# geloescht/mxnet-maintenance

Hardware: AMD Instinct MI355X
Metric: images/sec (whole node) ResNet-50 fp16 batch 256/GPU at 1/2/4/8 MI355X (higher is better)
Workload: dtype fp16; 1 GPU; model=ResNet-50 v1b, global_batch=256, per_gpu_batch=256, image_size=224, parallelism=dp1, layout=NHWC, optimizer=mp-SGD momentum 0.9, lr 0.1 (linear warm-up 40 steps), hip_graph=True, deterministic=True

## Files before the change

mxnet_maintenance_amd/ops/kernel_fns.py:

```python
import os

import torch

from . import kernels as _K
from .. import _state
from ..utils import env as _env

__all__ = ['BatchNormNHWC', 'BatchNormDualTailNHWC', 'SoftmaxCE', 'GlobalAvgPoolNHWC', 'flat_sgd']

_DT = {torch.float32: 0, torch.float16: 1, torch.bfloat16: 2}


def _stream():
    return torch.cuda.current_stream().cuda_stream


def _p(t):
    return 0 if t is None else t.data_ptr()


def _f32(t):
    if t.dtype == torch.float32 and t.is_contiguous():
        return t
    m = getattr(t, '_mxamd_master', None)
# ... 93 lines not shown
        C = x.shape[-1]
        R = x.numel() // C
        dev = x.device
        assert pool is None or (relu and addend is None)
        y = torch.empty_like(x) if pool is None else None
        if addend is not None:
            assert addend.shape == x.shape and addend.dtype == x.dtype
            addend = addend.contiguous()
        g, mean, invstd, var, scale, shift, args, host_update = _bn_fwd_stats(
            lib, x, gamma, beta, moving_mean, moving_var, eps, training, momentum)
        mask = (torch.empty(x.numel() // 8, dtype=torch.uint8, device=dev)
                if (addend is not None and relu and _RELU_FROM_X[0]) else None)
        lib.bn_nhwc_forward(_DT[x.dtype], x.data_ptr(), _p(addend), _p(y), _p(mask), *args(relu))
        if host_update is not None:
            host_update()
        ctx.pool = None
        if pool is not None:
            (kh, kw), (sh, sw), (ph, pw) = pool
            N, H, W = x.shape[:3]
            Ho, Wo = _pool_out(H, kh, sh, ph, False), _pool_out(W, kw, sw, pw, False)
            y = torch.empty((N, Ho, Wo, C), dtype=x.dtype, device=dev)
            arg = torch.empty((N, Ho, Wo, C), dtype=torch.uint8, device=dev)
            ctx.pool = (N, H, W, C, Ho, Wo, kh, kw, sh, sw, ph, pw, 1)
            lib.pool_nhwc_forward_bnrelu(_DT[x.dtype], x.data_ptr(), y.data_ptr(), arg.data_ptr(), *ctx.pool,
                                         _stream(), scale.data_ptr(), shift.data_ptr())
            mask = arg
        relu_mode = 0 if not relu else (1 if not _RELU_FROM_X[0] else (3 if addend is not None else 2))
        if pool is not None:
            relu_mode = 2
        ctx.save_for_backward(x, y if relu_mode == 1 else mask, g, mean, invstd,
                              scale if relu_mode == 2 else None, shift if relu_mode == 2 else None)
        ctx.cfg = (relu_mode, bool(training), addend is not None, gamma.dtype, beta.dtype)
        ctx.tee_key = getattr(addend, '_mxamd_tee_key', None) if (addend is not None and relu_mode == 3) else None
        ctx.bn_token = None
        if training and relu_mode in (0, 2, 3) and _BN_BWD_FUSE[0] and pool is None:
            ctx.bn_token = _BnToken()
            y._mxamd_bn_src = (x, mean, scale if relu_mode == 2 else None, shift if relu_mode == 2 else None,
                               mask if relu_mode == 3 else None, relu_mode, ctx.bn_token)
        ctx.refs = (gamma, beta)
        ctx.add_src = None
        if relu_mode == 3 and training and _BN_BWD_FUSE[0] and _BN_TAIL_DS[0]:
            src = getattr(addend, '_mxamd_bn_src', None)
            if (src is not None and src[5] == 0 and tuple(src[0].shape) == tuple(x.shape)
                    and src[0].dtype == x.dtype and src[0].is_contiguous()):
                ctx.add_src = src
        third = invstd if (invstd_out and training) else var
        ctx.mark_non_differentiable(mean, third)
        ctx.set_materialize_grads(False)
        return y, mean, third

    @staticmethod
    def backward(ctx, gy, _gm, _gv):
        lib = _K.lib()
        x, y, g, mean, invstd, fscale, fshift = ctx.saved_tensors
        relu_mode, training, has_add, gdt, bdt = ctx.cfg
        gamma_ref, beta_ref = ctx.refs
        if gy is None:
            return (None,) * 12
        gy = gy.contiguous()
        C = x.shape[-1]
        R = x.numel() // C
        dev = x.device
        fused_pool = False
        if ctx.pool is not None:
            fused_pool = (x.dtype in (torch.float16, torch.bfloat16) and 256 % (C // 8) == 0
                          and hasattr(lib, 'bn_pool_backward') and _BN_POOL_BWD[0])
            if not fused_pool:
                gyd = torch.empty_like(x)
                lib.pool_nhwc_backward(_DT[x.dtype], 1, gy.data_ptr(), y.data_ptr(), gyd.data_ptr(), *ctx.pool,
                                       _stream())
                gy, y = gyd, None
        lazy_mask = None
        tok = ctx.bn_token
        if tok is not None and tok.lazy is not None:
            dy_l, mask_l, ver_l = tok.lazy
            tok.lazy = None
            if gy is dy_l and gy._version == ver_l and relu_mode == 0 and not has_add and ctx.pool is None:
                lazy_mask = mask_l
            else:
                gy = (gy - dy_l + _materialize_dz(dy_l, mask_l)).contiguous()
        dx = torch.empty_like(x)
        dz = torch.empty_like(x) if has_add else None
        ext = getattr(gy, '_mxamd_bn_bwd', None)
        ext_nblk = 0
        if (ext is not None and ctx.bn_token is not None and ext[2] is ctx.bn_token
                and ext[3] == gy._version):
            part, ext_nblk = ext[0], ext[1]
        else:
            nblk = lib.bn_partials_rows(R, C)
            part = torch.empty(2 * nblk * C, dtype=torch.float32, device=dev)
        out = torch.empty(5, C, dtype=torch.float32, device=dev)
        need_g, need_b = ctx.needs_input_grad[1], ctx.needs_input_grad[2]
        tg = _leaf_grad(gamma_ref, C) if need_g else None
        tb = _leaf_grad(beta_ref, C) if need_b else None
        direct = tb is not None and (tg is not None or not need_g) and (tg is not None or tb is not None)
        if direct:
            dg_buf = tg if tg is not None else torch.zeros(C, dtype=torch.float32, device=dev)
            dg_ptr, db_ptr, accum = dg_buf.data_ptr(), tb.data_ptr(), 1
        else:
            dg_ptr, db_ptr, accum = out[0].data_ptr(), out[1].data_ptr(), 0
        if fused_pool:
            N_, H_, W_, C_, Ho_, Wo_, kh, kw, sh, sw, ph, pw, _ = ctx.pool
            ppart = torch.empty(2 * lib.bn_pool_bwd_blocks() * C, dtype=torch.float32, device=dev)
            lib.bn_pool_backward(_DT[x.dtype], x.data_ptr(), gy.data_ptr(), y.data_ptr(), dx.data_ptr(), g.data_ptr(),
                                 mean.data_ptr(), invstd.data_ptr(), fscale.data_ptr(), fshift.data_ptr(),
                                 ppart.data_ptr(), dg_ptr, db_ptr, out[2].data_ptr(), N_, H_, W_, C_, Ho_, Wo_, kh, kw,
                                 sh, sw, ph, pw, 0, int(training), accum, _stream())
            if direct:
                return dx, None, None, None, None, None, None, None, None, None, None, None
            return (dx, out[0].to(gdt) if need_g else None, out[1].to(bdt) if need_b else None,
                    None, None, None, None, None, None, None, None, None)
        ymask = y if relu_mode == 3 else None
        y = y if relu_mode == 1 else None
        ds = ctx.add_src if dz is not None else None
        lazy = (dz is not None and ds is None and ymask is not None and ctx.tee_key is not None
                and lazy_shortcut_ok(ctx.tee_key))
        lazy_ds = (dz is not None and ds is not None and ymask is not None and _LAZY_DZ[0]
                   and isinstance(ds[6], _BnToken))
        if lazy or lazy_ds:
            dz = None
        kmode = relu_mode
        if lazy_mask is not None:
            kmode, ymask = 3, lazy_mask
        dkw = {}
        if ds is not None:
            ds_nblk = lib.bn_tail_ds_rows(R, C)
            ds_part = torch.empty(2 * ds_nblk * C, dtype=torch.float32, device=dev)
            dkw = dict(ds_z=ds[0].data_ptr(), ds_mean=ds[1].data_ptr(), ds_part=ds_part.data_ptr())
        lib.bn_nhwc_backward(_DT[x.dtype], x.data_ptr(), gy.data_ptr(), _p(y), _p(ymask), dx.data_ptr(), _p(dz),
                             g.data_ptr(),
                             mean.data_ptr(), invstd.data_ptr(), _p(fscale), _p(fshift), part.data_ptr(), dg_ptr,
                             db_ptr, out[2].data_ptr(), R, C, kmode, 0, int(training), accum, _stream(),
                             ext_nblk, **dkw)
        if ds is not None:
            if lazy_ds:
                gy._mxamd_bn_bwd = (ds_part, ds_nblk, ds[6], gy._version)
                ds[6].lazy = (gy, ymask, gy._version)
                dz = gy
            else:
                dz._mxamd_bn_bwd = (ds_part, ds_nblk, ds[6], dz._version)
        if lazy:
            gy._mxamd_lazy_mask = (ymask, gy._version)
            dz = gy
        if direct:
            dgamma = None
            dbeta = None
        else:
            dgamma = out[0].to(gdt) if need_g else None
            dbeta = out[1].to(bdt) if need_b else None
        return dx, dgamma, dbeta, dz, None, None, None, None, None, None, None, None


_DUAL_TAIL_USED = [0]


def _bn_param_grad_dst(gamma_ref, beta_ref, need_g, need_b, out, C, dev):
    tg = _leaf_grad(gamma_ref, C) if need_g else None
    tb = _leaf_grad(beta_ref, C) if need_b else None
    if tb is not None and (tg is not None or not need_g):
        dg_buf = tg if tg is not None else torch.zeros(C, dtype=torch.float32, device=dev)
        return dg_buf.data_ptr(), tb.data_ptr(), 1, True, dg_buf
    return out[0].data_ptr(), out[1].data_ptr(), 0, False, None


class BatchNormDualTailNHWC(torch.autograd.Function):

# ... 1173 lines not shown
_SIDE_DIRTY = set()


def join_side_streams():
    if not _SIDE_DIRTY:
        return
    for dev in list(_SIDE_DIRTY):
        torch.cuda.current_stream(dev).wait_stream(_SIDE_STREAMS[dev])
    _SIDE_DIRTY.clear()
    del _SIDE_KEEP[:]


def _wgrad_maybe_side(dy, x, w, w_ref, stride, pad):
    if not (_WGRAD_SIDE[0] and dy.is_cuda):
        return _wgrad(dy, x, w, w_ref, stride, pad)
    dev = dy.device.index
    side = _SIDE_STREAMS.get(dev)
    if side is None:
        side = _SIDE_STREAMS[dev] = torch.cuda.Stream(device=dev)
        from .. import engine
        engine.add_join_hook(join_side_streams)
    main = torch.cuda.current_stream(dev)
    side.wait_stream(main)
    with torch.cuda.stream(side):
        dw = _wgrad(dy, x, w, w_ref, stride, pad)
    _SIDE_KEEP.append((dy, x))
    _SIDE_DIRTY.add(dev)
    if dw is not None:
        main.wait_stream(side)
        dw.record_stream(main)
    return dw


class ConvNHWC(torch.autograd.Function):

    @staticmethod
    def forward(ctx, x, w, bias, stride, pad, dilate):
        key = ('fwd', tuple(x.shape), tuple(w.shape), tuple(stride), tuple(pad), x.dtype, bias is not None)
        cands = _fwd_candidates(x, w, stride, pad, bias)
        y = _select(key, cands, _fwd_default(x, w, stride), timing=_fwd_timing(cands))
        ctx.save_for_backward(x, w)
        ctx.stride, ctx.pad = stride, pad
        ctx.has_bias = bias is not None
        ctx.b_ref = bias
        ctx.w_ref = w
        ctx.bn_src = getattr(x, '_mxamd_bn_src', None)
        return y

    @staticmethod
    def backward(ctx, dy):
        x, w = ctx.saved_tensors
        dy = dy.contiguous()
        stride, pad = ctx.stride, ctx.pad
        dx = dw = db = None
        if ctx.needs_input_grad[1] and _WGRAD_SIDE[0]:
            dw = _wgrad_maybe_side(dy, x, w, ctx.w_ref, stride, pad)
        if ctx.needs_input_grad[0]:
            key = ('dgrad', tuple(x.shape), tuple(w.shape), tuple(stride), tuple(pad), x.dtype)
            if _bn_bwd_fusable(ctx.bn_src, x.shape):
                cands, timing = _dgrad_bn_candidates(dy, x, w, stride, pad, ctx.bn_src)
                dx = _select(key + ('bnbwd',), cands, _dgrad_default(w, stride), timing=timing)
            else:
                dx = _select(key, _dgrad_candidates(dy, x, w, stride, pad), _dgrad_default(w, stride))
        if ctx.needs_input_grad[1] and not _WGRAD_SIDE[0]:
            dw = _wgrad(dy, x, w, ctx.w_ref, stride, pad)
        if ctx.has_bias and ctx.needs_input_grad[2]:
            db = _conv_bias_grad(dy, ctx.b_ref)
        return dx, dw, db, None, None, None


def _conv_bias_grad(dy, b_ref):
    from .nlp_fns import bias_grad
    return bias_grad(dy.reshape(-1, dy.shape[-1]), b_ref, b_ref.dtype)


class ConvTeeNHWC(torch.autograd.Function):

    @staticmethod
    def forward(ctx, x, w, inplace_grad=False):
        stride, pad = (1, 1), (0, 0)
        key = ('fwd', tuple(x.shape), tuple(w.shape), stride, pad, x.dtype, False)
        cands = _fwd_candidates(x, w, stride, pad, None)
        y = _select(key, cands, _fwd_default(x, w, stride), timing=_fwd_timing(cands))
        ctx.save_for_backward(x, w)
        ctx.w_ref = w
        ctx.inplace_grad = inplace_grad
        ctx.bn_src = getattr(x, '_mxamd_bn_src', None)
        xp = x.view_as(x)
        xp._mxamd_tee_key = _tee_key(x, w, ctx.bn_src)
        return y, xp

    @staticmethod
    def backward(ctx, gy, gpass):
        x, w = ctx.saved_tensors
        K, C = w.shape[0], w.shape[3]
        dx = dw = None
        if gy is None:
            return gpass, None, None
        gy = gy.contiguous()
        if ctx.needs_input_grad[1] and _WGRAD_SIDE[0]:
# ... 239 lines not shown
```

src/kernels/bindings.cc:

```cpp
#include <hip/hip_runtime.h>
#include <pybind11/pybind11.h>
#include <pybind11/stl.h>

#include <cstdint>
#include <stdexcept>
#include <vector>

namespace py = pybind11;

namespace mxamd {
void bn_nhwc_forward(int dtype, const void* x, const void* addend, void* y, uint8_t* mask, const float* gamma,
                     const float* beta,
                     const float* center, float* part, float* mean, float* invstd, float* var, float* scale,
                     float* shift, int64_t R, int C, float eps, int training, int relu, int fix_gamma,
                     float momentum, float* mm_upd, float* mv_upd, int ext_nblk, hipStream_t s, const float* ascale,
                     const float* ashift);
void bn_nhwc_backward(int dtype, const void* x, const void* dy, const void* y, const uint8_t* mask, void* dx,
                      void* dz,
                      const float* gamma, const float* mean, const float* invstd, const float* fscale,
                      const float* fshift, float* part, float* dgamma, float* dbeta, float* coef, int64_t R, int C,
                      int relu_mode, int fix_gamma, int training, int accum, hipStream_t s, int ext_nblk, const void* ds_z, const float* ds_mean, float* ds_part);
int bn_partials_rows(int64_t R, int C);
int bn_tail_ds_rows(int64_t R, int C);
void gemm_nt(int dtype, const void* a, const void* b, const void* bias, const void* addend, void* c, int out_f32,
// ... 136 lines not shown
                         int ph, int pw, int dh, int dw, int dg, int rows, hipStream_t s);
void deform_im2col_nhwc(int dtype, const void* x, const void* off, const void* msk, void* cols, const int* g,
                        int ld_off, int ld_msk, hipStream_t s);
void deform_bwd_nhwc(int dtype, const void* x, const void* off, const void* msk, const void* gcols, float* gx,
                     void* goff, void* gmsk, const int* g, int ld_off, int ld_msk, hipStream_t s);
void conv_dw_fwd(int dtype, const void* x, const void* wt, const float* bias, void* y, const int* gm, hipStream_t s);
void conv_dw_dgrad(int dtype, const void* dy, const void* wt, void* dx, const int* gm, hipStream_t s);
void conv_dw_wgrad(int dtype, const void* x, const void* dy, float* slab, int nslice, int out_dtype, void* out,
                   int accum, const int* gm, hipStream_t s);
int ssd_loss_blocks(int rows);
void ssd_loss_fwd(int dtype, const void* cls, const void* loc, const float* cls_t, const float* loc_t,
                  const float* loc_m, int rows, int C1, float lambd, float* part, float* out, hipStream_t s);
void ssd_loss_bwd(int dtype, const void* cls, const void* loc, const float* cls_t, const float* loc_t,
                  const float* loc_m, const float* stats, const float* gout, int rows, int C1, float lambd, void* dcls,
                  void* dloc, hipStream_t s);
void multibox_target(int dtype, const float* anchors, const float* labels, const void* cls_pred, float* loc_target,
                     float* loc_mask, float* cls_target, float* match_iou, int* match_gt, uint32_t* key, int B, int A,
                     int L, int W, int C, float thr, float ignore_label, float neg_ratio, float neg_thresh,
                     int min_neg, float v0, float v1, float v2, float v3, hipStream_t s);
void slab_reduce(int out_dtype, float* slab, int splits, int64_t n, void* out, int accum, hipStream_t s);
void twobit_quantize(int dtype, const void* g, float* res, void* packed, int64_t n, float thr, hipStream_t s);
void twobit_dequantize_sum(const void* packed, int64_t row_bytes, int nrows, int64_t n, float thr, float* out,
                           hipStream_t s);
int conv_pw_stream_ok(int kin, int nout);
int conv_pw_stream_grid(int M, int kin, int nout, int ncu, int add);
int conv_pw_stream_slices(int kin, int nout);
void weight_taps_t(int elem_bytes, const void* w, void* out, int K, int RS, int C, int n, const int* src,
                   const int64_t* base, const int64_t* rstride, hipStream_t s);
void conv_pw_stream(int dtype, const void* x, const void* w, void* y, const void* zero, int M, int kin, int nout,
                    float* part, int grid, hipStream_t s, const void* addend, int wt, const void* bn_z,
                    const uint8_t* bn_mask, const float* bn_mean, const float* bn_scale, const float* bn_shift,
                    int bn_mode, const uint8_t* addend_mask);
int conv_pw_stream_bnb_ok(int kin, int nout, int add, int mode);
void conv_gen(int dtype, int mode, const void* src, const void* wsrc, const float* bias, void* dst, const int* geom,
              int splits, hipStream_t s);
void rnn_fwd_seq(int dtype, int mode, const float* gx, const void* h0, const float* c0, const void* whh,
                 const float* bhh, void* out, int ldo, float* cseq, float* save, int Tn, int N, int H, int reverse,
                 hipStream_t s);
void rnn_bwd_seq(int dtype, int mode, const void* whhT, const void* dy, int ldy, const float* dhT,
                 const float* save, const float* cseq, const float* c0, const void* h0, const void* out, int ldo,
                 void* dgh, void* dgx, float* dc, float* dhd, float* dh0, int Tn, int N, int H, int reverse,
                 hipStream_t s);
}

using namespace mxamd;

template <typename T>
static inline T* P(uintptr_t p) {
  return reinterpret_cast<T*>(p);
}
static inline hipStream_t S(uintptr_t s) { return reinterpret_cast<hipStream_t>(s); }
static inline hipStream_t S_(uintptr_t s) { return reinterpret_cast<hipStream_t>(s); }

static void check_launch(const char* name) {
  hipError_t e = hipGetLastError();
  if (e != hipSuccess) throw std::runtime_error(std::string(name) + ": " + hipGetErrorString(e));
}

PYBIND11_MODULE(_hip_kernels, m) {
  m.doc() = "gfx950 HIP kernels for mxnet_maintenance_amd";
  m.attr("arch") = "gfx950";

  m.def("bn_partials_rows", &bn_partials_rows);
  m.def("bn_tail_ds_rows", &bn_tail_ds_rows);
  m.def("bn_nhwc_stats", [](int dt, uintptr_t x, uintptr_t center, uintptr_t part, int64_t R, int C, uintptr_t s) {
    int nblk = bn_nhwc_stats(dt, P<const void>(x), P<const float>(center), P<float>(part), R, C, S(s), 512);
// ... 49 lines not shown
    gemm_nt(dt, P<void>(a), P<void>(b), P<void>(bias), P<void>(addend), P<void>(c), out_f32, M, N, K, lda, ldb, ldc,
            act, cfg, splits, P<float>(ws), S(s), bias_lowp);
    check_launch("gemm_nt");
  }, py::arg("dt"), py::arg("a"), py::arg("b"), py::arg("bias"), py::arg("addend"), py::arg("c"), py::arg("out_f32"),
     py::arg("M"), py::arg("N"), py::arg("K"), py::arg("lda"), py::arg("ldb"), py::arg("ldc"), py::arg("act"),
     py::arg("cfg"), py::arg("splits"), py::arg("ws"), py::arg("s"), py::arg("bias_lowp") = 0);
  m.def("weight_taps_t", [](int eb, uintptr_t w, uintptr_t out, int K, int RS, int C, std::vector<int> src,
                            std::vector<int64_t> base, std::vector<int64_t> rstride, uintptr_t s) {
    if (src.size() != base.size() || src.size() != rstride.size()) throw std::runtime_error("weight_taps_t: table sizes");
    weight_taps_t(eb, P<const void>(w), P<void>(out), K, RS, C, static_cast<int>(src.size()), src.data(), base.data(),
                  rstride.data(), S(s));
    check_launch("weight_taps_t");
  });
  m.def("conv_pw_stream_ok", &conv_pw_stream_ok);
  m.def("conv_pw_stream_slices", &conv_pw_stream_slices);
  m.def("conv_pw_stream_grid", [](int M, int kin, int nout, int ncu, int add) {
    return conv_pw_stream_grid(M, kin, nout, ncu, add);
  }, pybind11::arg("M"), pybind11::arg("kin"), pybind11::arg("nout"), pybind11::arg("ncu"), pybind11::arg("add") = 0);
  m.def("conv_pw_stream", [](int dt, uintptr_t x, uintptr_t w, uintptr_t y, uintptr_t zero, int M, int kin, int nout,
                             uintptr_t part, int grid, uintptr_t s, uintptr_t addend, int wt, uintptr_t bn_z,
                             uintptr_t bn_mask, uintptr_t bn_mean, uintptr_t bn_scale, uintptr_t bn_shift, int bn_mode,
                             uintptr_t addend_mask) {
    conv_pw_stream(dt, P<const void>(x), P<const void>(w), P<void>(y), P<const void>(zero), M, kin, nout,
                   P<float>(part), grid, S(s), P<const void>(addend), wt, P<const void>(bn_z), P<const uint8_t>(bn_mask),
                   P<const float>(bn_mean), P<const float>(bn_scale), P<const float>(bn_shift), bn_mode,
                   P<const uint8_t>(addend_mask));
    check_launch("conv_pw_stream");
  }, pybind11::arg("dt"), pybind11::arg("x"), pybind11::arg("w"), pybind11::arg("y"), pybind11::arg("zero"),
     pybind11::arg("M"), pybind11::arg("kin"), pybind11::arg("nout"), pybind11::arg("part"), pybind11::arg("grid"),
     pybind11::arg("s"), pybind11::arg("addend"), pybind11::arg("wt") = 0, pybind11::arg("bn_z") = 0,
     pybind11::arg("bn_mask") = 0, pybind11::arg("bn_mean") = 0, pybind11::arg("bn_scale") = 0,
     pybind11::arg("bn_shift") = 0, pybind11::arg("bn_mode") = 0, pybind11::arg("addend_mask") = 0);
  m.def("conv_pw_stream_bnb_ok", &conv_pw_stream_bnb_ok);
  m.def("conv_gen", [](int dt, int mode, uintptr_t src, uintptr_t wsrc, uintptr_t bias, uintptr_t dst,
                       std::vector<int> geom, int splits, uintptr_t s) {
    if (geom.size() != 22) throw std::runtime_error("conv_gen: geometry needs 22 ints");
    conv_gen(dt, mode, P<const void>(src), P<const void>(wsrc), P<const float>(bias), P<void>(dst), geom.data(),
             splits, S(s));
    check_launch("conv_gen");
  });
  m.def("rnn_fwd_seq", [](int dt, int mode, uintptr_t gx, uintptr_t h0, uintptr_t c0, uintptr_t whh, uintptr_t bhh,
                          uintptr_t out, int ldo, uintptr_t cseq, uintptr_t save, int T, int N, int H, int reverse,
                          uintptr_t s) {
    rnn_fwd_seq(dt, mode, P<const float>(gx), P<const void>(h0), P<const float>(c0), P<const void>(whh),
                P<const float>(bhh), P<void>(out), ldo, P<float>(cseq), P<float>(save), T, N, H, reverse, S(s));
    check_launch("rnn_fwd_seq");
  });
  m.def("rnn_bwd_seq", [](int dt, int mode, uintptr_t whhT, uintptr_t dy, int ldy, uintptr_t dhT, uintptr_t save,
                          uintptr_t cseq, uintptr_t c0, uintptr_t h0, uintptr_t out, int ldo, uintptr_t dgh,
                          uintptr_t dgx, uintptr_t dc, uintptr_t dhd, uintptr_t dh0, int T, int N, int H, int reverse,
                          uintptr_t s) {
    rnn_bwd_seq(dt, mode, P<const void>(whhT), P<const void>(dy), ldy, P<const float>(dhT), P<const float>(save),
                P<const float>(cseq), P<const float>(c0), P<const void>(h0), P<const void>(out), ldo, P<void>(dgh),
                P<void>(dgx), P<float>(dc), P<float>(dhd), P<float>(dh0), T, N, H, reverse, S(s));
    check_launch("rnn_bwd_seq");
  });
  m.def("gemm_nt_tile_n", &gemm_nt_tile_n);
  m.def("gemm_nt_tile_m", &gemm_nt_tile_m);
  m.def("slab_reduce", [](int odt, uintptr_t slab, int splits, int64_t n, uintptr_t out, int accum, uintptr_t s) {
    slab_reduce(odt, P<float>(slab), splits, n, P<void>(out), accum, S(s));
    check_launch("slab_reduce");
  });
  m.def("deform_im2col", [](int dt, uintptr_t x, uintptr_t off, uintptr_t msk, uintptr_t cols, std::vector<int> g,
                            uintptr_t s) {
    if (g.size() != 15 && g.size() != 16) throw std::runtime_error("deform_im2col: geometry needs 15 or 16 ints");
    const int rows = g.size() == 16 ? g[15] : 0;
// ... 443 lines not shown
```

src/kernels/bn_nhwc.hip:

```cpp
#include <cstdlib>
#include <stdexcept>

#include <algorithm>

#include "common.h"

namespace mxamd {

constexpr int kBnThreads = 256;

struct BnGeom {
  int tpr;
  int cb;
  int rpi;
};

static inline BnGeom bn_geom(int C) {
  BnGeom g;
  int v = C / 8;
  g.tpr = v;
  if (v > kBnThreads)
    for (g.tpr = kBnThreads; v % g.tpr != 0; --g.tpr) {
    }
  g.cb = g.tpr * 8;
// ... 521 lines not shown
                             const float* gamma, const float* mean, const float* invstd, const float* fscale,
                             const float* fshift, float* part, float* dgamma, float* dbeta, float* coef, int64_t R,
                             int C, int relu_mode, int fix_gamma, int training, int accum, hipStream_t s,
                             int ext_nblk, const void* ds_z, const float* ds_mean, float* ds_part) {
  BnGeom g = bn_geom(C);
  int nblk;
  int64_t rpb = bn_rows_per_block(R, C, g, &nblk);
  if (ext_nblk > 0) nblk = ext_nblk;
  dim3 grid(nblk, C / g.cb);
  float* p1 = part;
  float* p2 = part + static_cast<int64_t>(nblk) * C;
  const T* xa = static_cast<const T*>(x);
  const T* dya = static_cast<const T*>(dy);
  const T* ya = static_cast<const T*>(y);
  MXAMD_HOST_CHECK(relu_mode != kReluFromY || y != nullptr, "bn_nhwc_backward: relu mask from y needs y");
  MXAMD_HOST_CHECK(relu_mode != kReluFromX || (fscale && fshift), "bn_nhwc_backward: relu-from-x needs scale/shift");
  MXAMD_HOST_CHECK(relu_mode != kReluFromMask || mask != nullptr, "bn_nhwc_backward: relu-from-mask needs the mask");
#define RED(RL)                                                                                                \
  hipLaunchKernelGGL((bn_reduce_kernel<T, 1, RL>), grid, dim3(kBnThreads), 0, s, xa, dya, ya, mask, mean, fscale, \
                     fshift,                                                                                         \
                     p1, p2, R, C, g.tpr, g.rpi, rpb)
  if (ext_nblk > 0) {
  } else if (relu_mode == kReluFromY) RED(kReluFromY);
  else if (relu_mode == kReluFromX) RED(kReluFromX);
  else if (relu_mode == kReluFromMask) RED(kReluFromMask);
  else RED(kReluNone);
#undef RED
  float* A = coef;
  float* B = coef + C;
  float* Cc = coef + 2 * C;
  hipLaunchKernelGGL((bn_finalize_kernel<1>), dim3((C + kFinPerBlock - 1) / kFinPerBlock), dim3(kFinThreads), 0, s, p1, p2, nblk, C, R, mean, gamma, nullptr,
                     invstd, 0.f, dgamma, dbeta, A, B, Cc, nullptr, fix_gamma, training, 0.f, nullptr,
                     nullptr, accum);
  const int64_t nvec = R * C / 8;
  int blocks = static_cast<int>((nvec + kBnThreads - 1) / kBnThreads);
  if (blocks > 256 * 16) blocks = 256 * 16;
  T* dxa = static_cast<T*>(dx);
  T* dza = static_cast<T*>(dz);
  if (ds_z) {
    MXAMD_HOST_CHECK(relu_mode == kReluFromMask && ds_mean && ds_part,
                     "bn_nhwc_backward: shortcut statistics need the tail's mask mode and the BN's mean");
    int dnblk;
    const int64_t drpb = bn_rows_per_block(R, C, g, &dnblk, bn_tail_blocks(), 64);
    hipLaunchKernelGGL((bn_tail_bwd_ds_kernel<T>), dim3(dnblk, C / g.cb), dim3(kBnThreads), 0, s, xa, dya, mask, A, B,
                       Cc, dxa, dza, static_cast<const T*>(ds_z), ds_mean, ds_part,
                       ds_part + static_cast<int64_t>(dnblk) * C, R, C, g.tpr, g.rpi, drpb, bn_nt());
    return;
  }
#define BWD(RL, WD)                                                                                      \
  hipLaunchKernelGGL((bn_bwd_apply_kernel<T, RL, WD>), dim3(blocks), dim3(kBnThreads), 0, s, xa, dya, ya, mask, A, B, \
                     Cc, fscale, fshift, dxa, dza, nvec, C, bn_nt())
  if (relu_mode == kReluFromY) {
    if (dz) BWD(kReluFromY, true); else BWD(kReluFromY, false);
  } else if (relu_mode == kReluFromX) {
    if (dz) BWD(kReluFromX, true); else BWD(kReluFromX, false);
  } else if (relu_mode == kReluFromMask) {
    if (dz) BWD(kReluFromMask, true); else BWD(kReluFromMask, false);
  } else {
    if (dz) BWD(kReluNone, true); else BWD(kReluNone, false);
  }
#undef BWD
}

int bn_nhwc_stats(int dtype, const void* x, const float* center, float* part, int64_t R, int C, hipStream_t s,
                  int total_blocks) {
  MXAMD_HOST_CHECK(C % 8 == 0, "bn_nhwc: channels must be a multiple of 8");
// ... 117 lines not shown
                       accum);
}

void bn_nhwc_forward(int dtype, const void* x, const void* addend, void* y, uint8_t* mask, const float* gamma,
                     const float* beta,
                     const float* center, float* part, float* mean, float* invstd, float* var, float* scale,
                     float* shift, int64_t R, int C, float eps, int training, int relu, int fix_gamma,
                     float momentum, float* mm_upd, float* mv_upd, int ext_nblk, hipStream_t s, const float* ascale,
                     const float* ashift) {
  switch (dtype) {
    case kF16:
      bn_forward_impl<__half>(x, addend, y, mask, gamma, beta, center, part, mean, invstd, var, scale, shift, R, C, eps,
                              training, relu, fix_gamma, momentum, mm_upd, mv_upd, ext_nblk, s, ascale, ashift);
      break;
    case kBF16:
      bn_forward_impl<__hip_bfloat16>(x, addend, y, mask, gamma, beta, center, part, mean, invstd, var, scale, shift, R,
                                      C, eps, training, relu, fix_gamma, momentum, mm_upd, mv_upd, ext_nblk, s, ascale,
                                      ashift);
      break;
    default:
      bn_forward_impl<float>(x, addend, y, mask, gamma, beta, center, part, mean, invstd, var, scale, shift, R, C, eps,
                             training, relu, fix_gamma, momentum, mm_upd, mv_upd, ext_nblk, s, ascale, ashift);
  }
}

void bn_finalize_backward(const float* part, int nblk, int C, int64_t R, const float* mean, const float* gamma,
                          const float* invstd, float* dgamma, float* dbeta, float* coef, int fix_gamma, int training,
                          int accum, hipStream_t s) {
  hipLaunchKernelGGL((bn_finalize_kernel<1>), dim3((C + kFinPerBlock - 1) / kFinPerBlock), dim3(kFinThreads), 0, s, part,
                     part + static_cast<int64_t>(nblk) * C, nblk, C, R, mean, gamma, nullptr, invstd, 0.f, dgamma,
                     dbeta, coef, coef + C, coef + 2 * C, nullptr, fix_gamma, training, 0.f, nullptr, nullptr, accum);
}

void bn_nhwc_backward(int dtype, const void* x, const void* dy, const void* y, const uint8_t* mask, void* dx,
                      void* dz,
                      const float* gamma, const float* mean, const float* invstd, const float* fscale,
                      const float* fshift, float* part, float* dgamma, float* dbeta, float* coef, int64_t R, int C,
                      int relu_mode, int fix_gamma, int training, int accum, hipStream_t s, int ext_nblk,
                      const void* ds_z, const float* ds_mean, float* ds_part) {
  switch (dtype) {
    case kF16:
      bn_backward_impl<__half>(x, dy, y, mask, dx, dz, gamma, mean, invstd, fscale, fshift, part, dgamma, dbeta, coef, R,
                               C, relu_mode, fix_gamma, training, accum, s, ext_nblk, ds_z, ds_mean, ds_part);
      break;
    case kBF16:
      bn_backward_impl<__hip_bfloat16>(x, dy, y, mask, dx, dz, gamma, mean, invstd, fscale, fshift, part, dgamma, dbeta,
                                       coef, R, C, relu_mode, fix_gamma, training, accum, s, ext_nblk, ds_z, ds_mean,
                                       ds_part);
      break;
    default:
      bn_backward_impl<float>(x, dy, y, mask, dx, dz, gamma, mean, invstd, fscale, fshift, part, dgamma, dbeta, coef, R,
                              C, relu_mode, fix_gamma, training, accum, s, ext_nblk, ds_z, ds_mean, ds_part);
  }
}

}
```

Baseline: 12570 images/sec.

## Fuse 1x1 conv dgrad+wgrad with BN backward apply in one kernel

Adds a persistent MFMA kernel that computes dgrad and wgrad together for 1x1 stride-1 convolutions with Cin=64, Cout=256. It can also apply the following BatchNorm's backward elementwise step (mask, A/B/C coefficients) in its prologue, so BN backward writes only coefficients and skips materialising dx. The goal is to cut separate reads of dy and x and the extra BN dx write/read pass. The fused path is chosen by autotuning against the existing dgrad+wgrad pair. This adds a lazy hand-off protocol between the BN and conv autograd functions, a per-block fp32 weight-gradient slab that needs a reduction, and 134 KB of LDS per workgroup.

```diff
diff --git a/mxnet_maintenance_amd/ops/kernel_fns.py b/mxnet_maintenance_amd/ops/kernel_fns.py
--- a/mxnet_maintenance_amd/ops/kernel_fns.py
+++ b/mxnet_maintenance_amd/ops/kernel_fns.py
@@ -149,6 +149,7 @@
                               scale if relu_mode == 2 else None, shift if relu_mode == 2 else None)
         ctx.cfg = (relu_mode, bool(training), addend is not None, gamma.dtype, beta.dtype)
         ctx.tee_key = getattr(addend, '_mxamd_tee_key', None) if (addend is not None and relu_mode == 3) else None
+        ctx.bwd1x1 = getattr(x, '_mxamd_bwd1x1', None) if (relu_mode == 3 and training) else None
         ctx.bn_token = None
         if training and relu_mode in (0, 2, 3) and _BN_BWD_FUSE[0] and pool is None:
             ctx.bn_token = _BnToken()
@@ -196,7 +197,6 @@
                 lazy_mask = mask_l
             else:
                 gy = (gy - dy_l + _materialize_dz(dy_l, mask_l)).contiguous()
-        dx = torch.empty_like(x)
         dz = torch.empty_like(x) if has_add else None
         ext = getattr(gy, '_mxamd_bn_bwd', None)
         ext_nblk = 0
@@ -218,7 +218,8 @@
             dg_ptr, db_ptr, accum = out[0].data_ptr(), out[1].data_ptr(), 0
         if fused_pool:
             N_, H_, W_, C_, Ho_, Wo_, kh, kw, sh, sw, ph, pw, _ = ctx.pool
-            ppart = torch.empty(2 * lib.bn_pool_bwd_blocks() * C, dtype=torch.float32, device=dev)
+            dx = torch.empty_like(x)
+            ppart =torch.empty(2 * lib.bn_pool_bwd_blocks() * C, dtype=torch.float32, device=dev)
             lib.bn_pool_backward(_DT[x.dtype], x.data_ptr(), gy.data_ptr(), y.data_ptr(), dx.data_ptr(), g.data_ptr(),
                                  mean.data_ptr(), invstd.data_ptr(), fscale.data_ptr(), fshift.data_ptr(),
                                  ppart.data_ptr(), dg_ptr, db_ptr, out[2].data_ptr(), N_, H_, W_, C_, Ho_, Wo_, kh, kw,
@@ -244,11 +245,23 @@
             ds_nblk = lib.bn_tail_ds_rows(R, C)
             ds_part = torch.empty(2 * ds_nblk * C, dtype=torch.float32, device=dev)
             dkw = dict(ds_z=ds[0].data_ptr(), ds_mean=ds[1].data_ptr(), ds_part=ds_part.data_ptr())
-        lib.bn_nhwc_backward(_DT[x.dtype], x.data_ptr(), gy.data_ptr(), _p(y), _p(ymask), dx.data_ptr(), _p(dz),
-                             g.data_ptr(),
+        hand = None
+        if (ctx.bwd1x1 is not None and _LAZY_BN_APPLY[0] and relu_mode == 3 and lazy_mask is None and ds is None
+                and training and ymask is not None and gy.data_ptr() % 16 == 0):
+            hand = (ctx.bwd1x1[0] + ('apply', bool(lazy)), ctx.bwd1x1[1])
+        take = hand is not None and _joint_algo(hand[0]) == 'fused'
+        if take and dz is not None:
+            dz = _materialize_dz(gy, ymask) if ctx.needs_input_grad[3] else None
+        dx = None if take else torch.empty_like(x)
+        lib.bn_nhwc_backward(_DT[x.dtype], x.data_ptr(), gy.data_ptr(), _p(y), _p(ymask), _p(dx),
+                             0 if take else _p(dz), g.data_ptr(),
                              mean.data_ptr(), invstd.data_ptr(), _p(fscale), _p(fshift), part.data_ptr(), dg_ptr,
                              db_ptr, out[2].data_ptr(), R, C, kmode, 0, int(training), accum, _stream(),
                              ext_nblk, **dkw)
+        if hand is not None:
+            carrier = gy if take else dx
+            hand[1].lazy = (carrier, carrier._version, gy, x, ymask, out, hand[0], not take, bool(lazy))
+            dx = carrier
         if ds is not None:
             if lazy_ds:
                 gy._mxamd_bn_bwd = (ds_part, ds_nblk, ds[6], gy._version)
@@ -1488,6 +1501,129 @@
     return dw
 
 
+_LAZY_BN_APPLY = [True]
+_PW_BWD_USED = [0, 0]
+
+
+def _joint_algo(key):
+    k = _akey(key)
+    name = _ALGO.get(k)
+    if name is None:
+        _load_tuning_file()
+        name = _FILE_ALGO.get(repr(k))
+        if name is not None:
+            _ALGO[k] = name
+    return name
+
+
+def _bwd1x1_base(x, w, stride, pad):
+    K, R, S, C = w.shape
+    if not (_CONV_HIP and R == 1 and S == 1 and tuple(stride) == (1, 1) and tuple(pad) == (0, 0) and x.is_cuda
+            and x.dtype in (torch.float16, torch.bfloat16) and w.dtype == x.dtype and x.dim() == 4):
+        return None
+    lib = _K.lib()
+    if not (hasattr(lib, 'conv_pw_bwd') and lib.conv_pw_bwd_ok(int(C), int(K))):
+        return None
+    return ('bwd1x1', tuple(x.shape), tuple(w.shape), x.dtype)
+
+
+def pw_bwd_ok(dy, x, w):
+    return (_bwd1x1_base(x, w, (1, 1), (0, 0)) is not None and dy.dtype == x.dtype and dy.is_contiguous()
+            and x.is_contiguous() and w.is_contiguous() and dy.data_ptr() % 16 == 0 and x.data_ptr() % 16 == 0
+            and w.data_ptr() % 16 == 0 and tuple(dy.shape) == tuple(x.shape[:-1]) + (w.shape[0],)
+            and dy.numel() < 2 ** 31)
+
+
+def conv_pw_bwd(dy, x, w, w_ref, apply=None, max_blocks=None, out=None):
+    K, C = w.shape[0], w.shape[3]
+    M = dy.numel() // K
+    if not pw_bwd_ok(dy, x, w):
+        raise ValueError('conv_pw_bwd: needs Cin = 64, Cout = 256, contiguous 16-byte aligned f16 / bf16 operands')
+    lib = _K.lib()
+    blocks = int(max_blocks) if max_blocks else _num_cus(dy.device)
+    wt = _dgrad_weight(w)
+    dx = torch.empty(x.shape, dtype=x.dtype, device=x.device)
+    slab = torch.empty(blocks * K * C, dtype=torch.float32, device=x.device)
+    a = (0, 0, 0, 0, 0)
+    if apply is not None:
+        x3, mask, coef = apply
+        if not (x3.shape == dy.shape and x3.dtype == dy.dtype and x3.is_contiguous() and x3.data_ptr() % 16 == 0
+                and mask.dtype == torch.uint8 and mask.is_contiguous() and mask.numel() * 8 == dy.numel()
+                and coef.dtype == torch.float32 and coef.is_contiguous() and tuple(coef.shape) == (5, K)):
+            raise ValueError('conv_pw_bwd: apply = (x3 like dy, 1-bit mask, fp32 coefficients [5][256])')
+        a = (x3.data_ptr(), mask.data_ptr(), coef[2].data_ptr(), coef[3].data_ptr(), coef[4].data_ptr())
+    lib.conv_pw_bwd(_DT[dy.dtype], dy.data_ptr(), *a, x.data_ptr(), wt.data_ptr(), dx.data_ptr(), slab.data_ptr(),
+                    M, C, K, blocks, _stream())
+    _PW_BWD_USED[int(apply is not None)] += 1
+    tgt = out if out is not None else _leaf_grad(w_ref, dtype=w.dtype)
+    if tgt is not None:
+        assert tgt.is_contiguous() and tgt.numel() == K * C and tgt.dtype in _DT
+        lib.slab_reduce(_DT[tgt.dtype], slab.data_ptr(), blocks, K * C, tgt.data_ptr(), 1, _stream())
+        return dx, None
+    dw = torch.empty(w.shape, dtype=w.dtype, device=w.device)
+    lib.slab_reduce(_DT[dw.dtype], slab.data_ptr(), blocks, K * C, dw.data_ptr(), 0, _stream())
+    return dx, dw
+
+
+def _bn_dx_torch(x, dy, mask, A, B, Cc):
+    bits = ((mask.view(-1, 1) >> torch.arange(8, device=mask.device, dtype=torch.uint8)) & 1).view(dy.shape)
+    dz = torch.where(bits.bool(), dy.float(), torch.zeros((), dtype=torch.float32, device=dy.device))
+    return (A * dz + B * x.float() + Cc).to(x.dtype)
+
+
+def _bn_dx(x, dy, mask, coef):
+    if not (x.is_cuda and _K.available() and x.dtype in (torch.float16, torch.bfloat16)):
+        return _bn_dx_torch(x, dy, mask, coef[2], coef[3], coef[4])
+    dx = torch.empty_like(x)
+    C = x.shape[-1]
+    _K.lib().bn_bwd_apply(_DT[x.dtype], x.data_ptr(), dy.data_ptr(), mask.data_ptr(), coef[2].data_ptr(),
+                          dx.data_ptr(), x.numel() // C, C, _stream())
+    return dx
+
+
+def _bwd1x1_tune(jkey, dy, x, w, stride, pad, bn_src, rec):
+    fusable = _bn_bwd_fusable(bn_src, x.shape)
+    dkey = ('dgrad', tuple(x.shape), tuple(w.shape), tuple(stride), tuple(pad), x.dtype) + (('bnbwd',) if fusable
+                                                                                             else ())
+    wkey = ('wgrad', tuple(x.shape), tuple(w.shape), tuple(stride), tuple(pad), x.dtype)
+    dg, wg = _ALGO.get(_akey(dkey)), _ALGO.get(_akey(wkey))
+    if dg is None or wg is None:
+        return
+    if fusable:
+        dfn = dict(_dgrad_bn_candidates(dy, x, w, stride, pad, bn_src)[1]).get(dg)
+    else:
+        dfn = dict(_dgrad_candidates(dy, x, w, stride, pad)).get(dg)
+    wfn = dict(_wgrad_candidates(dy, x, w, stride, pad)).get(wg)
+    if dfn is None or wfn is None:
+        return
+    scratch = torch.zeros_like(w)
+    if rec is not None:
+        gy, x3, mask, coef, lazy_dz = rec
+
+        def pair():
+            _bn_dx(x3, gy, mask, coef)
+            wfn()
+            return dfn()
+
+        def fused():
+            if not lazy_dz:
+                _materialize_dz(gy, mask)
+            return conv_pw_bwd(gy, x, w, None, apply=(x3, mask, coef), out=scratch)[0]
+    else:
+        def pair():
+            wfn()
+            return dfn()
+
+        def fused():
+            return conv_pw_bwd(dy, x, w, None, out=scratch)[0]
+    if fusable:
+        fused = _charge_bn_bwd([('fused', fused)], bn_src[0])[0][1]
+    pname = '+'.join(sorted([dg, wg], key=lambda n_: not _is_vendor(n_)))
+    used = list(_PW_BWD_USED)
+    _select(jkey, [(pname, pair), ('fused', fused)], pname)
+    _PW_BWD_USED[:] = used
+
+
 class ConvNHWC(torch.autograd.Function):
 
     @staticmethod
@@ -1501,6 +1637,10 @@
         ctx.b_ref = bias
         ctx.w_ref = w
         ctx.bn_src = getattr(x, '_mxamd_bn_src', None)
+        base = _bwd1x1_base(x, w, stride, pad)
+        ctx.bwd1x1 = None
+        if base is not None:
+            ctx.bwd1x1 = y._mxamd_bwd1x1 = (base, _BnToken())
         return y
 
     @staticmethod
@@ -1509,6 +1649,35 @@
         dy = dy.contiguous()
         stride, pad = ctx.stride, ctx.pad
         dx = dw = db = None
+        jkey = rec = None
+        if ctx.bwd1x1 is not None:
+            base, tok = ctx.bwd1x1
+            hand, tok.lazy = tok.lazy, None
+            same = False
+            if hand is not None:
+                carrier, ver, gy_l, x3, mask, coef, akey, materialised, lazy_dz = hand
+                same = dy is carrier and dy._version == ver
+                if not materialised and not (same and _joint_algo(akey) == 'fused' and pw_bwd_ok(dy, x, w)
+                                             and not (ctx.has_bias and ctx.needs_input_grad[2])
+                                             and ctx.needs_input_grad[0] and ctx.needs_input_grad[1]
+                                             and not _WGRAD_SIDE[0]):
+                    dx3 = _bn_dx(x3, gy_l, mask, coef)
+                    dy = dx3 if same else (dy - gy_l + dx3).contiguous()
+                    same, materialised = False, True
+            if (ctx.needs_input_grad[0] and ctx.needs_input_grad[1] and not _WGRAD_SIDE[0]
+                    and pw_bwd_ok(dy, x, w)):
+                if hand is not None and same:
+                    jkey, rec = akey, (gy_l, x3, mask, coef, lazy_dz)
+                else:
+                    jkey = base + ('plain',)
+                if _joint_algo(jkey) == 'fused':
+                    if rec is not None and not materialised:
+                        dx, dw = conv_pw_bwd(gy_l, x, w, ctx.w_ref, apply=(x3, mask, coef))
+                    else:
+                        dx, dw = conv_pw_bwd(dy, x, w, ctx.w_ref)
+                    if ctx.has_bias and ctx.needs_input_grad[2]:
+                        db = _conv_bias_grad(dy, ctx.b_ref)
+                    return dx, dw, db, None, None, None
         if ctx.needs_input_grad[1] and _WGRAD_SIDE[0]:
             dw = _wgrad_maybe_side(dy, x, w, ctx.w_ref, stride, pad)
         if ctx.needs_input_grad[0]:
@@ -1522,6 +1691,9 @@
             dw = _wgrad(dy, x, w, ctx.w_ref, stride, pad)
         if ctx.has_bias and ctx.needs_input_grad[2]:
             db = _conv_bias_grad(dy, ctx.b_ref)
+        if (jkey is not None and _joint_algo(jkey) is None and _AUTOTUNE
+                and not torch.cuda.is_current_stream_capturing()):
+            _bwd1x1_tune(jkey, dy, x, w, stride, pad, ctx.bn_src, rec)
         return dx, dw, db, None, None, None
 
 
diff --git a/src/kernels/bindings.cc b/src/kernels/bindings.cc
--- a/src/kernels/bindings.cc
+++ b/src/kernels/bindings.cc
@@ -192,6 +192,12 @@
                     const uint8_t* bn_mask, const float* bn_mean, const float* bn_scale, const float* bn_shift,
                     int bn_mode, const uint8_t* addend_mask);
 int conv_pw_stream_bnb_ok(int kin, int nout, int add, int mode);
+void bn_bwd_apply(int dtype, const void* x, const void* dy, const uint8_t* mask, const float* coef, void* dx,
+                  int64_t R, int C, hipStream_t s);
+int conv_pw_bwd_ok(int cin, int cout);
+void conv_pw_bwd(int dtype, const void* dy, const void* x3, const uint8_t* mask, const float* A, const float* B,
+                 const float* Cc, const void* X, const void* wt, void* dX, float* slab, int64_t M, int cin, int cout,
+                 int blocks, hipStream_t s);
 void conv_gen(int dtype, int mode, const void* src, const void* wsrc, const float* bias, void* dst, const int* geom,
               int splits, hipStream_t s);
 void rnn_fwd_seq(int dtype, int mode, const float* gx, const void* h0, const float* c0, const void* whh,
@@ -307,6 +313,21 @@
      pybind11::arg("bn_mask") = 0, pybind11::arg("bn_mean") = 0, pybind11::arg("bn_scale") = 0,
      pybind11::arg("bn_shift") = 0, pybind11::arg("bn_mode") = 0, pybind11::arg("addend_mask") = 0);
   m.def("conv_pw_stream_bnb_ok", &conv_pw_stream_bnb_ok);
+  m.def("bn_bwd_apply", [](int dt, uintptr_t x, uintptr_t dy, uintptr_t mask, uintptr_t coef, uintptr_t dx, int64_t R,
+                           int C, uintptr_t s) {
+    bn_bwd_apply(dt, P<const void>(x), P<const void>(dy), P<const uint8_t>(mask), P<const float>(coef), P<void>(dx), R,
+                 C, S(s));
+    check_launch("bn_bwd_apply");
+  });
+  m.def("conv_pw_bwd_ok", &conv_pw_bwd_ok);
+  m.def("conv_pw_bwd", [](int dt, uintptr_t dy, uintptr_t x3, uintptr_t mask, uintptr_t A, uintptr_t B, uintptr_t Cc,
+                          uintptr_t X, uintptr_t wt, uintptr_t dX, uintptr_t slab, int64_t M, int cin, int cout,
+                          int blocks, uintptr_t s) {
+    conv_pw_bwd(dt, P<const void>(dy), P<const void>(x3), P<const uint8_t>(mask), P<const float>(A), P<const float>(B),
+                P<const float>(Cc), P<const void>(X), P<const void>(wt), P<void>(dX), P<float>(slab), M, cin, cout,
+                blocks, S(s));
+    check_launch("conv_pw_bwd");
+  });
   m.def("conv_gen", [](int dt, int mode, uintptr_t src, uintptr_t wsrc, uintptr_t bias, uintptr_t dst,
                        std::vector<int> geom, int splits, uintptr_t s) {
     if (geom.size() != 22) throw std::runtime_error("conv_gen: geometry needs 22 ints");
diff --git a/src/kernels/bn_nhwc.hip b/src/kernels/bn_nhwc.hip
--- a/src/kernels/bn_nhwc.hip
+++ b/src/kernels/bn_nhwc.hip
@@ -577,6 +577,10 @@
   hipLaunchKernelGGL((bn_finalize_kernel<1>), dim3((C + kFinPerBlock - 1) / kFinPerBlock), dim3(kFinThreads), 0, s, p1, p2, nblk, C, R, mean, gamma, nullptr,
                      invstd, 0.f, dgamma, dbeta, A, B, Cc, nullptr, fix_gamma, training, 0.f, nullptr,
                      nullptr, accum);
+  if (dx == nullptr) {
+    MXAMD_HOST_CHECK(dz == nullptr && ds_z == nullptr, "bn_nhwc_backward: coefficients only writes no gradient");
+    return;
+  }
   const int64_t nvec = R * C / 8;
   int blocks = static_cast<int>((nvec + kBnThreads - 1) / kBnThreads);
   if (blocks > 256 * 16) blocks = 256 * 16;
@@ -760,6 +764,23 @@
                      dbeta, coef, coef + C, coef + 2 * C, nullptr, fix_gamma, training, 0.f, nullptr, nullptr, accum);
 }
 
+void bn_bwd_apply(int dtype, const void* x, const void* dy, const uint8_t* mask, const float* coef, void* dx,
+                  int64_t R, int C, hipStream_t s) {
+  MXAMD_HOST_CHECK(C % 8 == 0 && x && dy && mask && coef && dx, "bn_bwd_apply: operands");
+  MXAMD_HOST_CHECK(dtype == kF16 || dtype == kBF16, "bn_bwd_apply: dtype must be f16 or bf16");
+  const int64_t nvec = R * C / 8;
+  int blocks = static_cast<int>((nvec + kBnThreads - 1) / kBnThreads);
+  if (blocks > 256 * 16) blocks = 256 * 16;
+  const float* none = nullptr;
+#define APPLY_ONLY(T)                                                                                              \
+  hipLaunchKernelGGL((bn_bwd_apply_kernel<T, kReluFromMask, false>), dim3(blocks), dim3(kBnThreads), 0, s,           \
+                     static_cast<const T*>(x), static_cast<const T*>(dy), static_cast<const T*>(nullptr), mask, coef, \
+                     coef + C, coef + 2 * C, none, none, static_cast<T*>(dx), static_cast<T*>(nullptr), nvec, C,     \
+                     bn_nt())
+  if (dtype == kF16) APPLY_ONLY(__half); else APPLY_ONLY(__hip_bfloat16);
+#undef APPLY_ONLY
+}
+
 void bn_nhwc_backward(int dtype, const void* x, const void* dy, const void* y, const uint8_t* mask, void* dx,
                       void* dz,
                       const float* gamma, const float* mean, const float* invstd, const float* fscale,
diff --git a/src/kernels/conv_pw_bwd.hip b/src/kernels/conv_pw_bwd.hip
--- /dev/null
+++ b/src/kernels/conv_pw_bwd.hip
@@ -0,0 +1,262 @@
+#include <stdexcept>
+
+#include "common.h"
+#include "mfma.h"
+
+namespace mxamd {
+
+namespace {
+
+typedef short v4s __attribute__((ext_vector_type(4)));
+typedef short v8s __attribute__((ext_vector_type(8)));
+typedef float f4_t __attribute__((ext_vector_type(4)));
+typedef uint32_t u32x4 __attribute__((ext_vector_type(4)));
+typedef __attribute__((address_space(3))) v4s lds_v4s;
+
+constexpr int kCin = 64, kCout = 256, kBM = 64;
+constexpr int kSub = 64 * 64 * 2;
+constexpr int kGImg = 4 * kSub;
+constexpr int kXImg = kSub;
+constexpr int kDxPitch = kCin * 2 + 16;
+constexpr int kDxImg = kBM * kDxPitch;
+constexpr int kBuf = kGImg + kXImg + kDxImg;
+constexpr int kWPitch = kCout * 2 + 16;
+constexpr int kWImg = kCin * kWPitch;
+constexpr int kSmem = 2 * kBuf + kWImg;
+static_assert(kSmem <= 160 * 1024, "LDS of one CU");
+
+__device__ __forceinline__ int swz(int row) { return (((row >> 1) & 1) << 1) | (((row >> 3) & 1) << 2); }
+
+__device__ __forceinline__ v8s tr_frag(const char* tile, int off) {
+  typedef __attribute__((address_space(3))) char lds_char;
+  lds_char* base = (lds_char*)(tile);
+  v4s lo = __builtin_amdgcn_ds_read_tr16_b64_v4i16((lds_v4s*)(base + off));
+  v4s hi = __builtin_amdgcn_ds_read_tr16_b64_v4i16((lds_v4s*)(base + off + 512));
+  return v8s{lo[0], lo[1], lo[2], lo[3], hi[0], hi[1], hi[2], hi[3]};
+}
+
+__device__ __forceinline__ u32x4 load_nt(const void* p) {
+  return __builtin_nontemporal_load(reinterpret_cast<const u32x4*>(p));
+}
+
+template <bool APPLY>
+struct Stage {
+  u32x4 dy[4];
+  u32x4 x3[APPLY ? 4 : 1];
+  uint32_t mb[APPLY ? 4 : 1];
+  u32x4 xin;
+};
+
+template <typename T, bool APPLY>
+__global__ void __launch_bounds__(512) conv_pw_bwd_kernel(const T* __restrict__ dy, const T* __restrict__ x3,
+                                                          const uint8_t* __restrict__ mask,
+                                                          const float* __restrict__ A, const float* __restrict__ B,
+                                                          const float* __restrict__ Cc, const T* __restrict__ X,
+                                                          const T* __restrict__ wt, T* __restrict__ dX,
+                                                          float* __restrict__ slab, int M) {
+  extern __shared__ __attribute__((aligned(1024))) char smem[];
+  const int tid = threadIdx.x;
+  const int lane = tid & 63;
+  const int wid = tid >> 6;
+  const int nchunks = (M + kBM - 1) / kBM;
+  const int bid = blockIdx.x, grid = gridDim.x;
+  const int cpb = (nchunks + grid - 1) / grid;
+  const int c0 = bid * cpb;
+  const int n = min(max(nchunks - c0, 0), cpb);
+
+  const int cg = tid & 31, r0 = tid >> 5;
+  const int xr = tid >> 3, xc = tid & 7;
+  float ka[8], kb[8], kc[8];
+#pragma unroll
+  for (int q = 0; q < 8; ++q) {
+    ka[q] = APPLY ? A[cg * 8 + q] : 0.f;
+    kb[q] = APPLY ? B[cg * 8 + q] : 0.f;
+    kc[q] = APPLY ? Cc[cg * 8 + q] : 0.f;
+  }
+
+  char* wimg = smem + 2 * kBuf;
+#pragma unroll
+  for (int i = 0; i < 4; ++i) {
+    const int e = tid + i * 512;
+    *reinterpret_cast<u32x4*>(wimg + (e >> 5) * kWPitch + (e & 31) * 16) =
+        *reinterpret_cast<const u32x4*>(wt + static_cast<int64_t>(e) * 8);
+  }
+
+  auto load = [&](Stage<APPLY>& s, int chunk) {
+    const int p0 = chunk * kBM;
+#pragma unroll
+    for (int i = 0; i < 4; ++i) {
+      const int p = min(p0 + r0 + 16 * i, M - 1);
+      const int64_t e = static_cast<int64_t>(p) * kCout + cg * 8;
+      s.dy[i] = load_nt(dy + e);
+      if (APPLY) {
+        s.x3[i] = load_nt(x3 + e);
+        s.mb[i] = mask[e >> 3];
+      }
+    }
+    s.xin = *reinterpret_cast<const u32x4*>(X + static_cast<int64_t>(min(p0 + xr, M - 1)) * kCin + xc * 8);
+  };
+
+  auto commit = [&](const Stage<APPLY>& s, int chunk, char* buf) {
+    const int p0 = chunk * kBM;
+#pragma unroll
+    for (int i = 0; i < 4; ++i) {
+      const int r = r0 + 16 * i;
+      Vec8<T> g;
+      g.raw = __builtin_bit_cast(uint4, s.dy[i]);
+      if (APPLY) {
+        Vec8<T> d = g, xv;
+        xv.raw = __builtin_bit_cast(uint4, s.x3[i]);
+#pragma unroll
+        for (int q = 0; q < 8; ++q) {
+#pragma clang fp contract(off)
+          const float dd = ((s.mb[i] >> q) & 1u) ? d.get(q) : 0.f;
+          const float t = ka[q] * dd;
+          g.set(q, fmaf(kb[q], xv.get(q), t) + kc[q]);
+        }
+      }
+      if (p0 + r >= M) g.raw = make_uint4(0u, 0u, 0u, 0u);
+      *reinterpret_cast<uint4*>(buf + (cg >> 3) * kSub + r * 128 + (((cg & 7) ^ swz(r)) << 4)) = g.raw;
+    }
+    u32x4 xv = s.xin;
+    if (p0 + xr >= M) xv = u32x4{0u, 0u, 0u, 0u};
+    *reinterpret_cast<u32x4*>(buf + kGImg + xr * 128 + ((xc ^ swz(xr)) << 4)) = xv;
+  };
+
+  const int pf = wid >> 1, ch = wid & 1;
+  const int grow = pf * 16 + (lane & 15);
+  const int gswz = swz(grow);
+  const int wrow0 = (ch * 32 + (lane & 15)) * kWPitch + (lane >> 4) * 16;
+  const int fg = lane >> 4, fq = (lane >> 2) & 3, fp = lane & 3;
+  const int frow = 8 * fg + fq;
+  auto frag_off = [&](int f) { return frow * 128 + ((((2 * f) + (fp >> 1)) ^ swz(frow)) << 4) + ((fp & 1) << 3); };
+  int foff[4], goff[2];
+#pragma unroll
+  for (int f = 0; f < 4; ++f) foff[f] = frag_off(f);
+#pragma unroll
+  for (int j = 0; j < 2; ++j) goff[j] = frag_off(2 * ch + j);
+
+  f4_t accw[4][2];
+#pragma unroll
+  for (int i = 0; i < 4; ++i)
+#pragma unroll
+    for (int j = 0; j < 2; ++j) accw[i][j] = f4_t{0.f, 0.f, 0.f, 0.f};
+
+  auto store_dx = [&](int chunk, const char* buf) {
+    const int p = chunk * kBM + xr;
+    if (p < M)
+      *reinterpret_cast<uint4*>(dX + static_cast<int64_t>(p) * kCin + xc * 8) =
+          *reinterpret_cast<const uint4*>(buf + kGImg + kXImg + xr * kDxPitch + xc * 16);
+  };
+
+  auto mfmas = [&](char* buf) {
+    f4_t accx[2] = {f4_t{0.f, 0.f, 0.f, 0.f}, f4_t{0.f, 0.f, 0.f, 0.f}};
+#pragma unroll
+    for (int s = 0; s < 8; ++s) {
+      const int c8 = (s & 1) * 4 + (lane >> 4);
+      const u32x4 gb = *reinterpret_cast<const u32x4*>(buf + (s >> 1) * kSub + grow * 128 + ((c8 ^ gswz) << 4));
+#pragma unroll
+      for (int f = 0; f < 2; ++f) {
+        const u32x4 wa = *reinterpret_cast<const u32x4*>(wimg + wrow0 + f * 16 * kWPitch + s * 64);
+        accx[f] = mfma::Op<T>::run(wa, gb, accx[f]);
+      }
+    }
+    const char* gsub = buf + pf * kSub;
+    const char* ximg = buf + kGImg;
+#pragma unroll
+    for (int kk = 0; kk < 64; kk += 32) {
+      v8s a[4], b[2];
+#pragma unroll
+      for (int j = 0; j < 2; ++j) b[j] = tr_frag(gsub, kk * 128 + goff[j]);
+#pragma unroll
+      for (int i = 0; i < 4; ++i) a[i] = tr_frag(ximg, kk * 128 + foff[i]);
+#pragma unroll
+      for (int i = 0; i < 4; ++i)
+#pragma unroll
+        for (int j = 0; j < 2; ++j) accw[i][j] = mfma::Op<T>::run(a[i], b[j], accw[i][j]);
+    }
+#pragma unroll
+    for (int f = 0; f < 2; ++f) {
+      const int c = ch * 32 + f * 16 + (lane >> 4) * 4;
+      *reinterpret_cast<uint2*>(buf + kGImg + kXImg + grow * kDxPitch + c * 2) =
+          mfma::Op<T>::pack4(accx[f][0], accx[f][1], accx[f][2], accx[f][3]);
+    }
+  };
+
+  auto step = [&](Stage<APPLY>& s, int j, int b) {
+    char* buf = smem + b * kBuf;
+    commit(s, c0 + j, buf);
+    if (j + 2 < n) load(s, c0 + j + 2);
+    __syncthreads();
+    if (j > 0) store_dx(c0 + j - 1, smem + (b ^ 1) * kBuf);
+    mfmas(buf);
+  };
+
+  Stage<APPLY> sa, sb;
+  if (n > 0) load(sa, c0);
+  if (n > 1) load(sb, c0 + 1);
+  for (int j = 0; j < n; j += 2) {
+    step(sa, j, 0);
+    if (j + 1 < n) step(sb, j + 1, 1);
+  }
+  if (n > 0) {
+    __syncthreads();
+    store_dx(c0 + n - 1, smem + ((n - 1) & 1) * kBuf);
+  }
+
+  float* out = slab + static_cast<int64_t>(bid) * (kCout * kCin);
+#pragma unroll
+  for (int i = 0; i < 4; ++i)
+#pragma unroll
+    for (int j = 0; j < 2; ++j) {
+      const int k = pf * 64 + (2 * ch + j) * 16 + (lane & 15);
+      *reinterpret_cast<f4_t*>(out + k * kCin + i * 16 + (lane >> 4) * 4) = accw[i][j];
+    }
+}
+
+template <typename T, bool APPLY>
+void launch_pw_bwd(const void* dy, const void* x3, const uint8_t* mask, const float* A, const float* B,
+                   const float* Cc, const void* X, const void* wt, void* dX, float* slab, int M, int blocks,
+                   hipStream_t s) {
+  static bool set = false;
+  if (!set) {
+    MXAMD_HOST_CHECK(hipFuncSetAttribute(reinterpret_cast<const void*>(&conv_pw_bwd_kernel<T, APPLY>),
+                                         hipFuncAttributeMaxDynamicSharedMemorySize, kSmem) == hipSuccess,
+                     "conv_pw_bwd: the kernel needs 134 KB of LDS");
+    set = true;
+  }
+  hipLaunchKernelGGL((conv_pw_bwd_kernel<T, APPLY>), dim3(blocks), dim3(512), kSmem, s, static_cast<const T*>(dy),
+                     static_cast<const T*>(x3), mask, A, B, Cc, static_cast<const T*>(X), static_cast<const T*>(wt),
+                     static_cast<T*>(dX), slab, M);
+}
+
+inline bool aligned16(const void* p) { return (reinterpret_cast<uintptr_t>(p) & 15u) == 0; }
+
+}
+
+int conv_pw_bwd_ok(int cin, int cout) { return cin == kCin && cout == kCout ? 1 : 0; }
+
+void conv_pw_bwd(int dtype, const void* dy, const void* x3, const uint8_t* mask, const float* A, const float* B,
+                 const float* Cc, const void* X, const void* wt, void* dX, float* slab, int64_t M, int cin, int cout,
+                 int blocks, hipStream_t s) {
+  MXAMD_HOST_CHECK(conv_pw_bwd_ok(cin, cout), "conv_pw_bwd: built for Cin = 64, Cout = 256 only");
+  MXAMD_HOST_CHECK(dtype == kF16 || dtype == kBF16, "conv_pw_bwd: dtype must be f16 or bf16");
+  MXAMD_HOST_CHECK(M >= 1 && M * kCout < (1ll << 31), "conv_pw_bwd: pixel count out of range");
+  MXAMD_HOST_CHECK(blocks >= 1 && blocks <= 4096, "conv_pw_bwd: workgroup count out of range");
+  MXAMD_HOST_CHECK(dy && X && wt && dX && slab && aligned16(dy) && aligned16(X) && aligned16(wt) && aligned16(dX) &&
+                       aligned16(slab),
+                   "conv_pw_bwd: operands must be non-null and 16-byte aligned");
+  const bool apply = x3 != nullptr;
+  MXAMD_HOST_CHECK(!apply || (mask && A && B && Cc && aligned16(x3)),
+                   "conv_pw_bwd: the BatchNorm prologue needs x3 (16-byte aligned), the mask and A / B / Cc");
+  const int m = static_cast<int>(M);
+  if (dtype == kF16) {
+    if (apply) launch_pw_bwd<__half, true>(dy, x3, mask, A, B, Cc, X, wt, dX, slab, m, blocks, s);
+    else launch_pw_bwd<__half, false>(dy, x3, mask, A, B, Cc, X, wt, dX, slab, m, blocks, s);
+  } else {
+    if (apply) launch_pw_bwd<__hip_bfloat16, true>(dy, x3, mask, A, B, Cc, X, wt, dX, slab, m, blocks, s);
+    else launch_pw_bwd<__hip_bfloat16, false>(dy, x3, mask, A, B, Cc, X, wt, dX, slab, m, blocks, s);
+  }
+}
+
+}
```

New measurement: 12960 images/sec (median of 6 runs). +3.1%, better.
